# Yxxxb/LAVT-RS

Measured on NVIDIA B200. Metric: LAVT-RS fwd clips/s (8x384^2), higher is better.
Workload: dtype bf16

## Files before the change

### include/lavt_b200.h

```cpp
#ifndef LAVT_B200_H_
#define LAVT_B200_H_

#include <stdint.h>

#ifdef __cplusplus
extern "C" {
#endif

#define LAVT_ABI_VERSION 4

#define LAVT_ERR_SHAPE 1
#define LAVT_ERR_CUDA 2
#define LAVT_ERR_ARCH 3

enum { LAVT_ACT_NONE = 0, LAVT_ACT_GELU = 1, LAVT_ACT_RELU = 2, LAVT_ACT_TANH = 3, LAVT_ACT_SIGMOID = 4 };

typedef struct lavt_win_geom {
  int32_t B, D, H, W;
  int32_t wd, wh, ww;
  int32_t sd, sh, sw;
  int32_t nwd, nwh, nww;
  int32_t N;
  int32_t Wd, Wh, Ww;
} lavt_win_geom_t;

typedef struct lavt_epilogue {
  const float* cscale;
  const float* bias;
  int32_t act;
  int32_t ldm;
  const void* mul;
  const float* resid;
// ... 4 lines not shown
  const lavt_win_geom_t* win;
  const float* rscale;
  int32_t rscale_rows;
  int32_t pre_mode;
  void* out_pre;
} lavt_epilogue_t;

const char* lavt_last_error(void);
int lavt_abi_version(void);
int lavt_check_device(void);

int lavt_gemm_bf16(const void* A, int64_t lda, const void* Wt, int64_t ldw, int32_t M, int32_t N, int32_t K,
                   const lavt_epilogue_t* epi, void* stream);

int lavt_conv3x3_bf16(const void* x_nhwc, int64_t ldx, int32_t n_img, int32_t H, int32_t W, int32_t Cin,
                      const void* Wt, int32_t Cout, const lavt_epilogue_t* epi, void* stream);

int lavt_conv3d_bf16(const void* x_ndhwc, int64_t ldx, int32_t n_clip, int32_t D, int32_t H, int32_t W, int32_t Cin,
                     const void* Wt, int32_t Cout, const lavt_epilogue_t* epi, void* stream);


int lavt_layernorm_rows(const float* x, int64_t ldx, int64_t M, int32_t C, const float* gamma, const float* beta,
                        float eps, void* out_bf16, float* out_f32, void* stream);

int lavt_layernorm_window_gather(const float* x, int32_t C, const lavt_win_geom_t* geom, const float* gamma,
                                 const float* beta, float eps, void* out_bf16, void* stream);

int lavt_patch_merge_layernorm(const float* x, int32_t B, int32_t D, int32_t H, int32_t W, int32_t C,
                               const float* gamma, const float* beta, float eps, void* out_bf16, void* stream);

int lavt_patch_embed_im2col(const float* x, int64_t stride_b, int64_t stride_c, int64_t stride_t, int32_t B, int32_t T,
                            int32_t H, int32_t W, void* out_bf16, void* stream);

int lavt_window_attention(const void* qkv, const float* table_t, int32_t L, int32_t nH, const lavt_win_geom_t* geom,
                          void* out_bf16, void* stream);
int lavt_window_attention_lse(const void* qkv, const float* table_t, int32_t L, int32_t nH, const lavt_win_geom_t* geom, void* out_bf16,
                              float* lse, void* stream);
int lavt_window_attention_has_lse(const lavt_win_geom_t* geom, int32_t L, int32_t nH);
int lavt_set_attention_impl(int32_t impl);

int64_t lavt_instnorm_workspace_floats(int32_t B, int64_t n, int32_t C);
int lavt_instnorm_stats(const float* x, int32_t B, int64_t n, int32_t C, float eps, float* stats,
                        float* workspace, void* stream);
int lavt_pwam_kv(const float* l, const float* mask, const float* wk, const float* bk, const float* wv, const float* bv,
                 float* k, float* v, int32_t B, int32_t Nl, int32_t Lin, int32_t C, void* stream);
int lavt_lang_project(const float* l, const float* mask, const float* w0, const float* b0, const float* w2, const float* b2, float* stats,
// ... 157 lines not shown
```

### lavt_rs_b200/_cabi.py

```python
from __future__ import annotations

import ctypes as C
import os
from typing import Optional

import torch

_PKG = os.path.dirname(os.path.abspath(__file__))
LIB_PATH = os.environ.get("LAVT_LIB_PATH") or os.path.join(_PKG, "_lib", "liblavt_b200.so")

ACT_NONE, ACT_GELU, ACT_RELU, ACT_TANH, ACT_SIGMOID = 0, 1, 2, 3, 4


class WinGeom(C.Structure):
    _fields_ = [(n, C.c_int32) for n in
                ("B", "D", "H", "W", "wd", "wh", "ww", "sd", "sh", "sw",
                 "nwd", "nwh", "nww", "N", "Wd", "Wh", "Ww")]

    def rows(self) -> int:
        return self.B * self.nwd * self.nwh * self.nww * self.N

    def tokens(self) -> int:
        return self.B * self.D * self.H * self.W

# ... 15 lines not shown
    pass


_lib: Optional[C.CDLL] = None


def lib() -> C.CDLL:
    global _lib
    if _lib is not None:
        return _lib
    if not os.path.exists(LIB_PATH):
        raise LavtError(
            f"{LIB_PATH} not found: build it with `python -m lavt_rs_b200.build` "
            "(the B200 path has no CPU / PyTorch fallback)")
    l = C.CDLL(LIB_PATH)
    l.lavt_last_error.restype = C.c_char_p
    _declare(l)
    if l.lavt_abi_version() != ABI_VERSION:
        raise LavtError("liblavt_b200.so ABI version mismatch; rebuild")
    _lib = l
    return l


ABI_VERSION = 4

_i32, _i64, _f32, _vp = C.c_int32, C.c_int64, C.c_float, C.c_void_p
_EP = C.POINTER(Epilogue)
_WG = C.POINTER(WinGeom)

SIGNATURES = {
    "lavt_check_device": [],
    "lavt_gemm_bf16": [_vp, _i64, _vp, _i64, _i32, _i32, _i32, _EP, _vp],
    "lavt_gemm_bf16_smallm": [_vp, _i64, _vp, _i64, _i32, _i32, _i32, _EP, _vp, _i64, _vp],
    "lavt_conv3x3_bf16": [_vp, _i64, _i32, _i32, _i32, _i32, _vp, _i32, _EP, _vp],
    "lavt_conv3d_bf16": [_vp, _i64, _i32, _i32, _i32, _i32, _i32, _vp, _i32, _EP, _vp],
    "lavt_layernorm_rows": [_vp, _i64, _i64, _i32, _vp, _vp, _f32, _vp, _vp, _vp],
    "lavt_layernorm_window_gather": [_vp, _i32, _WG, _vp, _vp, _f32, _vp, _vp],
    "lavt_patch_merge_layernorm": [_vp, _i32, _i32, _i32, _i32, _i32, _vp, _vp, _f32, _vp, _vp],
    "lavt_patch_embed_im2col": [_vp, _i64, _i64, _i64, _i32, _i32, _i32, _i32, _vp, _vp],
    "lavt_window_attention": [_vp, _vp, _i32, _i32, _WG, _vp, _vp],
    "lavt_window_attention_lse": [_vp, _vp, _i32, _i32, _WG, _vp, _vp, _vp],
    "lavt_instnorm_stats": [_vp, _i32, _i64, _i32, _f32, _vp, _vp, _vp],
    "lavt_pwam_kv": [_vp, _vp, _vp, _vp, _vp, _vp, _vp, _vp, _i32, _i32, _i32, _i32, _vp],
    "lavt_lang_project": [_vp, _vp, _vp, _vp, _vp, _vp, _vp, _i32, _i32, _i32, _i32, _vp],
    "lavt_lang_project_bwd": [_vp, _vp, _vp, _vp, _vp, _vp, _vp, _vp, _vp, _vp, _vp, _vp, _i32, _i32, _i32, _i32, _vp],
    "lavt_pwam_attend": [_vp, _vp, _vp, _vp, _vp, _vp, _i32, _i64, _i32, _i32, _i32, _vp],
    "lavt_pwam_mul_norm": [_vp, _vp, _vp, _vp, _i32, _i64, _i32, _vp],
    "lavt_instnorm_sum2": [_vp, _vp, _vp, _vp, _vp, _i32, _i64, _i32, _vp],
    "lavt_bert_embed": [_vp, _vp, _vp, _vp, _vp, _i32, _i32, _i32, _i32, _vp],
    "lavt_bert_attention": [_vp, _vp, _vp, _i32, _i32, _i32, _i32, _vp],
    "lavt_rows_to_channels_first": [_vp, _vp, _i32, _i32, _i32, _vp],
    "lavt_split3_bf16": [_vp, _i64, _vp, _i64, _i32, _vp],
    "lavt_bert_attention_f32": [_vp, _vp, _vp, _i32, _i32, _i32, _i32, _vp],
    "lavt_upsample_concat": [_vp, _i32, _i32, _i32, _vp, _i32, _vp, _i32, _i32, _i32, _vp],
    "lavt_upconv_blend": [_vp, _i32, _i32, _i32, _vp, _vp, _vp, _vp, _i32, _i32, _i32, _vp],
    "lavt_conv1x1_logits": [_vp, _vp, _vp, _vp, _i64, _i32, _vp],
    "lavt_upsample_logits": [_vp, _vp, _i32, _i32, _i32, _i32, _i32, _vp],
    "lavt_nhwc_to_nchw": [_vp, _vp, _i32, _i32, _i32, _vp],
    "lavt_nchw_to_nhwc_bf16": [_vp, _vp, _i32, _i32, _i32, _vp],
# ... 254 lines not shown
    npos = n_clip * D * H * W
    TIMER.end(t0, "gemm_bf16_tc_kernel", 2.0 * npos * Cout * 27 * Cin, 2.0 * (npos * Cin + Cout * 27 * Cin + npos * Cout),
              f"conv3d {n_clip}x{D}x{H}x{W} Cin{Cin} Cout{Cout}")


def _c(t: torch.Tensor, dtype, name: str) -> torch.Tensor:
    _req(t, dtype, name)
    if not t.is_contiguous():
        raise LavtError(f"{name} must be contiguous")
    return t


def layernorm_rows(x: torch.Tensor, gamma, beta, *, out_bf16=None, out_f32=None, eps: float = 1e-5) -> None:
    _req(x, torch.float32, "x")
    M, Cn = x.shape
    for t, dt, nm in ((out_bf16, torch.bfloat16, "out_bf16"), (out_f32, torch.float32, "out_f32")):
        if t is not None:
            _c(t, dt, nm)
    check(lib().lavt_layernorm_rows(x.data_ptr(), x.stride(0), M, Cn, _c(gamma, torch.float32, "gamma").data_ptr(),
                                    _c(beta, torch.float32, "beta").data_ptr(), eps, ptr(out_bf16), ptr(out_f32),
                                    stream_ptr()), "lavt_layernorm_rows")


def layernorm_window_gather(x: torch.Tensor, geom: WinGeom, gamma, beta, out_bf16: torch.Tensor, eps: float = 1e-5) -> None:
    _c(x, torch.float32, "x")
    Cn = x.shape[-1]
    if x.numel() != geom.tokens() * Cn or out_bf16.numel() != geom.rows() * Cn:
        raise LavtError("window gather: tensor sizes do not match the geometry")
    check(lib().lavt_layernorm_window_gather(x.data_ptr(), Cn, C.byref(geom), _c(gamma, torch.float32, "gamma").data_ptr(),
                                             _c(beta, torch.float32, "beta").data_ptr(), eps,
                                             _c(out_bf16, torch.bfloat16, "out").data_ptr(), stream_ptr()),
          "lavt_layernorm_window_gather")


def patch_merge_layernorm(x: torch.Tensor, B, D, H, W, gamma, beta, out_bf16: torch.Tensor, eps: float = 1e-5) -> None:
    _c(x, torch.float32, "x")
    Cn = x.shape[-1]
    check(lib().lavt_patch_merge_layernorm(x.data_ptr(), B, D, H, W, Cn, _c(gamma, torch.float32, "gamma").data_ptr(),
                                           _c(beta, torch.float32, "beta").data_ptr(), eps,
                                           _c(out_bf16, torch.bfloat16, "out").data_ptr(), stream_ptr()),
          "lavt_patch_merge_layernorm")


def patch_embed_im2col(x: torch.Tensor, out_bf16: torch.Tensor) -> None:
    _req(x, torch.float32, "x")
    B, Cin, T, H, W = x.shape
# ... 725 lines not shown
```

### lavt_rs_b200/csrc/cabi.cu

```cuda
#include "../../include/lavt_b200.h"
#include "common.cuh"
#include "gemm_tc.cuh"
#include "kernels.cuh"

#include <cstring>

namespace lavt {
const char* last_error();
int gemm_dispatch(const void* A, long long lda, const void* Bw, long long ldb, const GemmParams& p,
                  cudaStream_t stream);

static_assert(sizeof(lavt_win_geom_t) == sizeof(WinGeom), "public/private window geometry mismatch");

static int fill_epilogue(GemmParams& p, const lavt_epilogue_t* e) {
  LAVT_REQUIRE(e != nullptr, "epilogue pointer is NULL");
  p.cscale = e->cscale;
  p.bias = e->bias;
  p.act = e->act;
  p.mul = static_cast<const __nv_bfloat16*>(e->mul);
  p.ldm = e->ldm;
  p.mul_act = e->mul_act;
  p.out_pre = static_cast<__nv_bfloat16*>(e->out_pre);
  p.pre_mode = e->pre_mode;
  LAVT_REQUIRE(e->pre_mode == 0 || (e->pre_mode == 1 && e->out_pre && e->act == LAVT_ACT_GELU),
// ... 87 lines not shown
  p.M = n_clip * D * H * W; p.N = Cout; p.K = 27 * Cin;
  int rc = fill_epilogue(p, epi);
  if (rc) return rc;
  LAVT_REQUIRE(p.rowmap == ROWMAP_IDENTITY, "conv3d: window row map not applicable");
  p.rowmap = ROWMAP_CONV;
  p.cH = H; p.cW = W; p.cCin = Cin; p.taps = 27; p.cD = D;
  conv_pick_tile(p, H, W);
  return gemm_dispatch(x_ndhwc, ldx, Wt, 27LL * Cin, p, static_cast<cudaStream_t>(stream));
}

static inline cudaStream_t S(void* s) { return static_cast<cudaStream_t>(s); }
static inline const __nv_bfloat16* CB(const void* p) { return static_cast<const __nv_bfloat16*>(p); }
static inline __nv_bfloat16* MB(void* p) { return static_cast<__nv_bfloat16*>(p); }

int lavt_layernorm_rows(const float* x, int64_t ldx, int64_t M, int32_t C, const float* gamma, const float* beta,
                        float eps, void* out_bf16, float* out_f32, void* stream) {
  LnParams p;
  std::memset(&p, 0, sizeof(p));
  p.x = x; p.ldx = ldx; p.gamma = gamma; p.beta = beta; p.out_bf16 = MB(out_bf16); p.out_f32 = out_f32;
  p.M = M; p.C = C; p.eps = eps;
  return ln_rows_dispatch(MODE_IDENTITY, p, S(stream));
}

int lavt_layernorm_window_gather(const float* x, int32_t C, const lavt_win_geom_t* geom, const float* gamma,
                                 const float* beta, float eps, void* out_bf16, void* stream) {
  LAVT_REQUIRE(geom != nullptr, "window gather: geometry is NULL");
  LnParams p;
  std::memset(&p, 0, sizeof(p));
  std::memcpy(&p.win, geom, sizeof(WinGeom));
  p.x = x; p.ldx = C; p.gamma = gamma; p.beta = beta; p.out_bf16 = MB(out_bf16);
  p.M = 1LL * geom->B * geom->nwd * geom->nwh * geom->nww * geom->N; p.C = C; p.eps = eps;
  return ln_rows_dispatch(MODE_WINDOW, p, S(stream));
}

int lavt_patch_merge_layernorm(const float* x, int32_t B, int32_t D, int32_t H, int32_t W, int32_t C,
                               const float* gamma, const float* beta, float eps, void* out_bf16, void* stream) {
  LnParams p;
  std::memset(&p, 0, sizeof(p));
  p.x = x; p.ldx = C; p.gamma = gamma; p.beta = beta; p.out_bf16 = MB(out_bf16);
  p.M = 1LL * B * D * ((H + 1) / 2) * ((W + 1) / 2); p.C = C; p.eps = eps;
  p.mB = B; p.mD = D; p.mH = H; p.mW = W;
  return ln_rows_dispatch(MODE_MERGE, p, S(stream));
}

int lavt_patch_embed_im2col(const float* x, int64_t stride_b, int64_t stride_c, int64_t stride_t, int32_t B, int32_t T,
                            int32_t H, int32_t W, void* out_bf16, void* stream) {
// ... 443 lines not shown
```

### lavt_rs_b200/csrc/common.cuh

```cuda
#pragma once

#include <cuda.h>
#include <cuda_bf16.h>
#include <cuda_runtime.h>
#include <stdint.h>
#include <string.h>

#define LAVT_OK 0
#define LAVT_ERR_SHAPE 1
#define LAVT_ERR_CUDA 2
#define LAVT_ERR_ARCH 3

namespace lavt {

void set_last_error(const char* fmt, ...);
int check_cuda(cudaError_t e, const char* what);
#define LAVT_CUDA(call)                                   \
  do {                                                    \
    int _rc = ::lavt::check_cuda((call), #call);          \
    if (_rc != LAVT_OK) return _rc;                       \
  } while (0)
#define LAVT_LAUNCH_CHECK(name)                           \
  do {                                                    \
    int _rc = ::lavt::check_cuda(cudaGetLastError(), name); \
// ... 67 lines not shown
#pragma unroll
  for (int o = 16; o > 0; o >>= 1) v += __shfl_xor_sync(0xffffffffu, v, o);
  return v;
}
__device__ __forceinline__ float warp_max(float v) {
#pragma unroll
  for (int o = 16; o > 0; o >>= 1) v = fmaxf(v, __shfl_xor_sync(0xffffffffu, v, o));
  return v;
}

__device__ __forceinline__ uint32_t pack_bf16x2(float lo, float hi) {
  __nv_bfloat162 v = __floats2bfloat162_rn(lo, hi);
  return *reinterpret_cast<uint32_t*>(&v);
}
__device__ __forceinline__ float2 unpack_bf16x2(uint32_t u) {
  __nv_bfloat162 v = *reinterpret_cast<__nv_bfloat162*>(&u);
  return __bfloat1622float2(v);
}

__device__ __forceinline__ float gelu_erf(float x) {
  return 0.5f * x * (1.0f + erff(x * 0.70710678118654752440f));
}

__device__ __forceinline__ void mbar_init(uint64_t* bar, uint32_t count) {
  asm volatile("mbarrier.init.shared::cta.b64 [%0], %1;" ::"r"(smem_u32(bar)), "r"(count));
}
__device__ __forceinline__ void fence_mbar_init() {
  asm volatile("fence.mbarrier_init.release.cluster;" ::: "memory");
}
__device__ __forceinline__ void mbar_expect_tx(uint64_t* bar, uint32_t bytes) {
  asm volatile("mbarrier.arrive.expect_tx.shared::cta.b64 _, [%0], %1;" ::"r"(smem_u32(bar)),
               "r"(bytes)
               : "memory");
}
__device__ __forceinline__ void mbar_arrive(uint64_t* bar) {
  asm volatile("mbarrier.arrive.shared::cta.b64 _, [%0];" ::"r"(smem_u32(bar)) : "memory");
}
__device__ __forceinline__ bool mbar_try_wait(uint64_t* bar, uint32_t parity) {
  uint32_t ok;
  asm volatile(
      "{\n\t"
      ".reg .pred P;\n\t"
      "mbarrier.try_wait.parity.shared::cta.b64 P, [%1], %2, %3;\n\t"
      "selp.u32 %0, 1, 0, P;\n\t"
      "}\n"
      : "=r"(ok)
// ... 242 lines not shown
```

### lavt_rs_b200/csrc/gemm_tc.cu

```cuda
#include "common.cuh"
#include "gemm_tc.cuh"

#include <cstdio>
#include <cstdlib>
#include <cstring>

namespace lavt {

constexpr int GEMM_BM = 128;
constexpr int GEMM_BK = 64;

template <int GEMM_BN, int GEMM_STAGES, int EPI_WGS, int CTA2 = 0>
struct GemmSmem {
  static constexpr int A_BYTES = GEMM_BM * GEMM_BK * 2;
  static constexpr int B_BYTES = (CTA2 ? GEMM_BN / 2 : GEMM_BN) * GEMM_BK * 2;
  static constexpr int STAGE_BYTES = A_BYTES + B_BYTES;
  static constexpr int RING_BYTES = GEMM_STAGES * STAGE_BYTES;
  static constexpr int BAR_OFF = RING_BYTES;
  static constexpr int VEC_OFF = BAR_OFF + 256;
  static constexpr int VEC_TILE_BYTES = EPI_WGS * 2 * GEMM_BN * 4;
  static constexpr int TOTAL = VEC_OFF + VEC_TILE_BYTES + 1024 ;
  static constexpr int THREADS = 128 + 128 * EPI_WGS;
  static constexpr int MIN_CTAS = (EPI_WGS == 1) ? 2 : 1;
  static constexpr int ACC = (MIN_CTAS == 2) ? 2 : 512 / GEMM_BN;
};

__device__ __forceinline__ float ex2_approx(float x) {
  float y;
  asm("ex2.approx.ftz.f32 %0, %1;" : "=f"(y) : "f"(x));
  return y;
}
__device__ __forceinline__ float rcp_approx(float x) {
  float y;
  asm("rcp.approx.ftz.f32 %0, %1;" : "=f"(y) : "f"(x));
  return y;
}
__device__ __forceinline__ uint64_t pk2(float lo, float hi) {
  uint64_t r;
  asm("mov.b64 %0, {%1, %2};" : "=l"(r) : "f"(lo), "f"(hi));
  return r;
}
__device__ __forceinline__ void upk2(uint64_t v, float& lo, float& hi) { asm("mov.b64 {%0, %1}, %2;" : "=f"(lo), "=f"(hi) : "l"(v)); }
__device__ __forceinline__ uint64_t fma2(uint64_t a, uint64_t b, uint64_t c) {
  uint64_t r;
  asm("fma.rn.f32x2 %0, %1, %2, %3;" : "=l"(r) : "l"(a), "l"(b), "l"(c));
  return r;
}
__device__ __forceinline__ uint64_t mul2(uint64_t a, uint64_t b) {
  uint64_t r;
  asm("mul.rn.f32x2 %0, %1, %2;" : "=l"(r) : "l"(a), "l"(b));
  return r;
}
__device__ __forceinline__ void gelu_erf2(float& x0, float& x1) {
  const uint64_t x = pk2(x0, x1);
  float z0, z1;
  upk2(mul2(x, pk2(0.70710678118654752f, 0.70710678118654752f)), z0, z1);
  z0 = fminf(fmaxf(z0, -3.0f), 3.0f);
  z1 = fminf(fmaxf(z1, -3.0f), 3.0f);
  const uint64_t z = pk2(z0, z1);
  const uint64_t t = mul2(z, z);
  constexpr float K = 1.0000220904f;
  uint64_t p = pk2(4.0742095563e-08f * K, 4.0742095563e-08f * K);
  p = fma2(p, t, pk2(-1.9448222676e-06f * K, -1.9448222676e-06f * K));
  p = fma2(p, t, pk2(4.1060515983e-05f * K, 4.1060515983e-05f * K));
  p = fma2(p, t, pk2(-5.1103678896e-04f * K, -5.1103678896e-04f * K));
  p = fma2(p, t, pk2(4.2354270142e-03f * K, 4.2354270142e-03f * K));
  p = fma2(p, t, pk2(-2.5102860078e-02f * K, -2.5102860078e-02f * K));
  p = fma2(p, t, pk2(1.1107933337e-01f * K, 1.1107933337e-01f * K));
  p = fma2(p, t, pk2(-3.7531487405e-01f * K, -3.7531487405e-01f * K));
  p = fma2(p, t, pk2(1.1282684285e+00f * K, 1.1282684285e+00f * K));
  const uint64_t e = mul2(z, p);
  const uint64_t hx = mul2(x, pk2(0.5f, 0.5f));
  upk2(fma2(hx, e, hx), x0, x1);
}
__device__ __forceinline__ void gelu_both2(float& x0, float& x1, float& d0, float& d1) {
  const uint64_t x = pk2(x0, x1);
  float z0, z1;
  upk2(mul2(x, pk2(0.70710678118654752f, 0.70710678118654752f)), z0, z1);
  const uint64_t zz = pk2(z0, z1);
  float q0, q1;
  upk2(mul2(zz, zz), q0, q1);
  const float e0 = ex2_approx(-1.4426950408889634f * q0), e1 = ex2_approx(-1.4426950408889634f * q1);
  z0 = fminf(fmaxf(z0, -3.0f), 3.0f);
  z1 = fminf(fmaxf(z1, -3.0f), 3.0f);
  const uint64_t z = pk2(z0, z1);
  const uint64_t t = mul2(z, z);
  constexpr float K = 1.0000220904f;
  uint64_t p = pk2(4.0742095563e-08f * K, 4.0742095563e-08f * K);
  p = fma2(p, t, pk2(-1.9448222676e-06f * K, -1.9448222676e-06f * K));
  p = fma2(p, t, pk2(4.1060515983e-05f * K, 4.1060515983e-05f * K));
  p = fma2(p, t, pk2(-5.1103678896e-04f * K, -5.1103678896e-04f * K));
  p = fma2(p, t, pk2(4.2354270142e-03f * K, 4.2354270142e-03f * K));
  p = fma2(p, t, pk2(-2.5102860078e-02f * K, -2.5102860078e-02f * K));
  p = fma2(p, t, pk2(1.1107933337e-01f * K, 1.1107933337e-01f * K));
  p = fma2(p, t, pk2(-3.7531487405e-01f * K, -3.7531487405e-01f * K));
  p = fma2(p, t, pk2(1.1282684285e+00f * K, 1.1282684285e+00f * K));
  const uint64_t Phi = fma2(mul2(z, p), pk2(0.5f, 0.5f), pk2(0.5f, 0.5f));
  const uint64_t xs = mul2(x, pk2(0.3989422804014327f, 0.3989422804014327f));
  upk2(fma2(xs, pk2(e0, e1), Phi), d0, d1);
  upk2(mul2(x, Phi), x0, x1);
}
__device__ __forceinline__ void gelu_grad2(float& x0, float& x1) {
  float d0, d1;
  gelu_both2(x0, x1, d0, d1);
  x0 = d0;
  x1 = d1;
}
__device__ __forceinline__ void ldg_v8(uint32_t* r, const void* p) {
  asm volatile("ld.global.v8.b32 {%0, %1, %2, %3, %4, %5, %6, %7}, [%8];"
               : "=r"(r[0]), "=r"(r[1]), "=r"(r[2]), "=r"(r[3]), "=r"(r[4]), "=r"(r[5]), "=r"(r[6]), "=r"(r[7])
               : "l"(p));
}
__device__ __forceinline__ void stg_v8(void* p, const uint32_t* r) {
  asm volatile("st.global.v8.b32 [%0], {%1, %2, %3, %4, %5, %6, %7, %8};" ::"l"(p), "r"(r[0]), "r"(r[1]), "r"(r[2]),
               "r"(r[3]), "r"(r[4]), "r"(r[5]), "r"(r[6]), "r"(r[7])
               : "memory");
}
__device__ __forceinline__ float tanh_fast(float x) {
  const float e = ex2_approx(x * 2.8853900817779268f);
  return fmaf(-2.0f, rcp_approx(e + 1.0f), 1.0f);
}

template <int GEMM_BN, int GEMM_STAGES, int EPI_WGS, int CTA2 = 0, int SIMPLE = 0>
__global__ void __launch_bounds__(GemmSmem<GEMM_BN, GEMM_STAGES, EPI_WGS, CTA2>::THREADS, GemmSmem<GEMM_BN, GEMM_STAGES, EPI_WGS, CTA2>::MIN_CTAS)
gemm_bf16_tc_kernel(const __grid_constant__ CUtensorMap tmA, const __grid_constant__ CUtensorMap tmB,
                    const GemmParams p, const int m_tiles, const int vec_all, long long* const trace_buf) {
  using L = GemmSmem<GEMM_BN, GEMM_STAGES, EPI_WGS, CTA2>;
  const int crank = CTA2 ? static_cast<int>(cluster_ctarank()) : 0;
  const int wid0 = CTA2 ? static_cast<int>(blockIdx.x >> 1) : static_cast<int>(blockIdx.x);
  const int wstep = CTA2 ? static_cast<int>(gridDim.x >> 1) : static_cast<int>(gridDim.x);
  extern __shared__ uint8_t smem_raw[];
  uint8_t* smem = smem_raw + ((1024u - (smem_u32(smem_raw) & 1023u)) & 1023u);
  uint64_t* full_bar = reinterpret_cast<uint64_t*>(smem + L::BAR_OFF);
  uint64_t* empty_bar = full_bar + GEMM_STAGES;
  constexpr int ACC = L::ACC;
  uint64_t* tmem_full_bar = empty_bar + GEMM_STAGES;
  uint64_t* tmem_empty_bar = tmem_full_bar + ACC;
  uint32_t* tmem_ptr_smem = reinterpret_cast<uint32_t*>(tmem_empty_bar + ACC);

  const int warp = threadIdx.x >> 5;
// ... 568 lines not shown
```

### lavt_rs_b200/csrc/kernels.cuh

```cuda
#pragma once
#include "common.cuh"
#include "geom.cuh"

namespace lavt {

enum { MODE_IDENTITY = 0, MODE_WINDOW = 1, MODE_MERGE = 2 };

struct LnParams {
  const float* x;
  long long ldx;
  const float* gamma;
  const float* beta;
  __nv_bfloat16* out_bf16;
  float* out_f32;
  long long M;
  int C;
  float eps;
  WinGeom win;
  int mB, mD, mH, mW;
};
int ln_rows_dispatch(int mode, const LnParams& p, cudaStream_t st);
int im2col_patch4_dispatch(const float* x, long long sB, long long sC, long long sT, __nv_bfloat16* out, int B, int T, int H,
                           int W, cudaStream_t st);
long long colstats_workspace_floats(int B, long long n, int C);
// ... 99 lines not shown
int pwam_kv_bwd_dispatch(const float* dkbuf, const float* dvbuf, const float* mask, const float* l, const float* wk, const float* wv,
                         float* dwk, float* dbk, float* dwv, float* dbv, float* dl, int B, int Nl, int NlPad, int Lin, int C, int heads,
                         cudaStream_t st);
int gate_elem_dispatch(int mode, const __nv_bfloat16* a, const __nv_bfloat16* b, const float* f, const float* f2, __nv_bfloat16* out_bf16,
                       float* out_f32, long long count, cudaStream_t st);

int pwam_kv_dispatch(const float* l, const float* mask, const float* wk, const float* bk, const float* wv, const float* bv,
                     float* k, float* v, int B, int Nl, int Lin, int C, cudaStream_t st);
int lang_project_dispatch(const float* l, const float* mask, const float* w0, const float* b0, const float* w2, const float* b2,
                          float* stats, int B, int Nl, int Lin, int C, cudaStream_t st);
int pwam_core_dispatch(const float* qpre, const float* stats, const float* k, const float* v, const float* mask,
                       __nv_bfloat16* o, int B, long long n, int C, int Nl, int heads, cudaStream_t st);

int bert_embed_dispatch(const long long* ids, const float* word, const float* pos, const float* type0, float* out, int B, int Nl,
                        int H, int vocab, cudaStream_t st);
int bert_attention_dispatch(const __nv_bfloat16* qkv, const float* mask, __nv_bfloat16* out, int B, int Nl, int H, int heads,
                            cudaStream_t st);
int split3_bf16_dispatch(const float* x, long long ldx, __nv_bfloat16* out, long long M, int Kd, cudaStream_t st);
int bert_attention_f32_dispatch(const float* qkv, const float* mask, float* out, int B, int Nl, int H, int heads, cudaStream_t st);
int rows_to_cf_dispatch(const float* in, float* out, int B, int Nl, int C, cudaStream_t st);

int upsample_concat_dispatch(const __nv_bfloat16* prev, int ph, int pw, int C1, const __nv_bfloat16* skip, int C2,
                             __nv_bfloat16* out, int n_img, int H, int W, cudaStream_t st);
int upconv_blend_dispatch(const __nv_bfloat16* Z, int h, int w, int hid, const float* P, const float* s, const float* b,
                          __nv_bfloat16* out, int n_img, int H, int W, cudaStream_t st);
int conv1x1_logits_dispatch(const __nv_bfloat16* y, const float* w, const float* b, float* out, long long npix, int C,
                            cudaStream_t st);
int upsample_logits_dispatch(const float* in, float* out, int n_img, int h, int w, int H, int W, cudaStream_t st);
int nhwc_to_nchw_dispatch(const float* in, float* out, int n_img, int P, int C, cudaStream_t st);
int nchw_to_nhwc_bf16_dispatch(const float* in, __nv_bfloat16* out, int n_img, int P, int C, cudaStream_t st);

}
```

### lavt_rs_b200/engine.py

```python
from __future__ import annotations

from typing import Dict, Optional, Sequence, Tuple

import torch

from . import _cabi as K
from .geometry import window_geometry

LAUNCHES = 0
PRECISION = "bf16"


def set_precision(mode: str) -> str:
    global PRECISION
    if mode not in ("bf16", "fp32"):
        raise ValueError("precision must be 'bf16' or 'fp32'")
    prev, PRECISION = PRECISION, mode
    return prev


def _count(n: int = 1) -> None:
    global LAUNCHES
    LAUNCHES += n

# ... 73 lines not shown
    if PRECISION == "fp32":
        return _swin_block_fp32(x, blk, geom, ws, xb_out)

    qkv_w = pw.get("qkv_w", [blk.attn.qkv.weight], lambda: _bf16(blk.attn.qkv.weight))
    def _qscale():
        s = torch.ones(3 * C, device=dev, dtype=torch.float32)
        s[:C] = hd ** -0.5 * 1.4426950408889634
        b = _f32(blk.attn.qkv.bias) * s if blk.attn.qkv.bias is not None else torch.zeros(3 * C, device=dev)
        return s, b
    qkv_s, qkv_b = pw.get("qkv_sb", [blk.attn.qkv.weight] + ([blk.attn.qkv.bias] if blk.attn.qkv.bias is not None else []), _qscale)
    proj_w = pw.get("proj_w", [blk.attn.proj.weight], lambda: _bf16(blk.attn.proj.weight))
    fc1_w = pw.get("fc1_w", [blk.mlp.fc1.weight], lambda: _bf16(blk.mlp.fc1.weight))
    fc2_w = pw.get("fc2_w", [blk.mlp.fc2.weight], lambda: _bf16(blk.mlp.fc2.weight))
    table_t = pw.get("table_t", [blk.attn.relative_position_bias_table],
                     lambda: _f32(blk.attn.relative_position_bias_table.t()))

    xw = ws.get("xw", (rows, C), torch.bfloat16, dev)
    K.layernorm_window_gather(x, geom, blk.norm1.weight, blk.norm1.bias, xw, eps=blk.norm1.eps)
    qkv = ws.get("qkv", (rows, 3 * C), torch.bfloat16, dev)
    K.gemm_bf16(xw, qkv_w, cscale=qkv_s, bias=qkv_b, out_bf16=qkv)
    att = ws.get("att", (rows, C), torch.bfloat16, dev)
    K.window_attention(qkv, table_t, geom, att)
    K.gemm_bf16(att, proj_w, bias=blk.attn.proj.bias.detach(), resid=x, out_f32=x, win=geom)
    h1 = ws.get("ln2", (n, C), torch.bfloat16, dev)
    K.layernorm_rows(x, blk.norm2.weight, blk.norm2.bias, out_bf16=h1, eps=blk.norm2.eps)
    hid = ws.get("hid", (n, fc1_w.shape[0]), torch.bfloat16, dev)
    K.gemm_bf16(h1, fc1_w, bias=blk.mlp.fc1.bias.detach(), act=K.ACT_GELU, out_bf16=hid)
    K.gemm_bf16(hid, fc2_w, bias=blk.mlp.fc2.bias.detach(), resid=x, out_f32=x, out_bf16=xb_out)
    _count(7)


def _swin_block_fp32(x: torch.Tensor, blk, geom, ws: Workspace, xb_out: Optional[torch.Tensor]) -> None:
    n, C = x.shape
    dev = x.device
    rows, nH = geom.rows(), blk.num_heads
    hd = C // nH
    s = torch.ones(3 * C, device=dev, dtype=torch.float32)
    s[:C] = hd ** -0.5 * 1.4426950408889634
    qb = _f32(blk.attn.qkv.bias) * s if blk.attn.qkv.bias is not None else torch.zeros(3 * C, device=dev)
    xw = ws.get("xw32", (rows, C), torch.float32, dev)
    K.layernorm_window_gather_f32(x, geom, blk.norm1.weight, blk.norm1.bias, xw, eps=blk.norm1.eps)
    qkv = ws.get("qkv32", (rows, 3 * C), torch.float32, dev)
    K.gemm_f32_ref(xw, _f32(blk.attn.qkv.weight), cscale=s, bias=qb, out_f32=qkv)
    att = ws.get("att32", (rows, C), torch.float32, dev)
    K.window_attention_f32_ref(qkv, _f32(blk.attn.relative_position_bias_table.t()), geom, att)
    K.gemm_f32_ref(att, _f32(blk.attn.proj.weight), bias=blk.attn.proj.bias.detach(), resid=x, out_f32=x, win=geom)
    h1 = ws.get("ln2_32", (n, C), torch.float32, dev)
    K.layernorm_rows(x, blk.norm2.weight, blk.norm2.bias, out_f32=h1, eps=blk.norm2.eps)
    hid = ws.get("hid32", (n, blk.mlp.fc1.weight.shape[0]), torch.float32, dev)
    K.gemm_f32_ref(h1, _f32(blk.mlp.fc1.weight), bias=blk.mlp.fc1.bias.detach(), act=K.ACT_GELU, out_f32=hid)
    K.gemm_f32_ref(hid, _f32(blk.mlp.fc2.weight), bias=blk.mlp.fc2.bias.detach(), resid=x, out_f32=x, out_bf16=xb_out)
# ... 690 lines not shown
```

Baseline: 298.1.

## Fuse Swin MLP LayerNorm, fc1+GELU, fc2 and residual into one tcgen05 kernel

Adds a persistent warp-specialized kernel for C=256 Swin blocks. It computes LayerNorm2 into shared memory, runs fc1 into TMEM, applies GELU and feeds the hidden tile back from TMEM as the A operand of fc2, then adds bias and residual in place. This removes the global round-trip of the 4C-wide hidden activation and the LN output, and drops two launches per block. The price is a complex pipeline with a 640-thread, single-CTA-per-SM configuration, and only the C=256 stage uses it.

```diff
diff --git a/include/lavt_b200.h b/include/lavt_b200.h
--- a/include/lavt_b200.h
+++ b/include/lavt_b200.h
@@ -7,7 +7,7 @@
 extern "C" {
 #endif
 
-#define LAVT_ABI_VERSION 4
+#define LAVT_ABI_VERSION 5
 
 #define LAVT_ERR_SHAPE 1
 #define LAVT_ERR_CUDA 2
@@ -58,6 +58,9 @@
 
 int lavt_layernorm_rows(const float* x, int64_t ldx, int64_t M, int32_t C, const float* gamma, const float* beta,
                         float eps, void* out_bf16, float* out_f32, void* stream);
+
+int lavt_swin_mlp(float* x, int64_t M, int32_t C, int32_t H, const float* ln_w, const float* ln_b, float eps, const void* w1_bf16,
+                  const float* b1, const void* w2_bf16, const float* b2, void* xb_out, void* stream);
 
 int lavt_layernorm_window_gather(const float* x, int32_t C, const lavt_win_geom_t* geom, const float* gamma,
                                  const float* beta, float eps, void* out_bf16, void* stream);
diff --git a/lavt_rs_b200/_cabi.py b/lavt_rs_b200/_cabi.py
--- a/lavt_rs_b200/_cabi.py
+++ b/lavt_rs_b200/_cabi.py
@@ -61,7 +61,7 @@
     return l
 
 
-ABI_VERSION = 4
+ABI_VERSION = 5
 
 _i32, _i64, _f32, _vp = C.c_int32, C.c_int64, C.c_float, C.c_void_p
 _EP = C.POINTER(Epilogue)
@@ -74,6 +74,7 @@
     "lavt_conv3x3_bf16": [_vp, _i64, _i32, _i32, _i32, _i32, _vp, _i32, _EP, _vp],
     "lavt_conv3d_bf16": [_vp, _i64, _i32, _i32, _i32, _i32, _i32, _vp, _i32, _EP, _vp],
     "lavt_layernorm_rows": [_vp, _i64, _i64, _i32, _vp, _vp, _f32, _vp, _vp, _vp],
+    "lavt_swin_mlp": [_vp, _i64, _i32, _i32, _vp, _vp, _f32, _vp, _vp, _vp, _vp, _vp, _vp],
     "lavt_layernorm_window_gather": [_vp, _i32, _WG, _vp, _vp, _f32, _vp, _vp],
     "lavt_patch_merge_layernorm": [_vp, _i32, _i32, _i32, _i32, _i32, _vp, _vp, _f32, _vp, _vp],
     "lavt_patch_embed_im2col": [_vp, _i64, _i64, _i64, _i32, _i32, _i32, _i32, _vp, _vp],
@@ -374,6 +375,24 @@
                                     stream_ptr()), "lavt_layernorm_rows")
 
 
+def swin_mlp(x: torch.Tensor, ln_w, ln_b, eps: float, w1: torch.Tensor, b1, w2: torch.Tensor, b2, *, xb_out=None) -> None:
+    _c(x, torch.float32, "x")
+    M, Cn = x.shape
+    Hn = _c(w1, torch.bfloat16, "w1").shape[0]
+    if tuple(w1.shape) != (Hn, Cn) or tuple(_c(w2, torch.bfloat16, "w2").shape) != (Cn, Hn):
+        raise LavtError(f"swin_mlp: w1 {tuple(w1.shape)} / w2 {tuple(w2.shape)} do not match C = {Cn}")
+    for t, n in ((b1, Hn), (b2, Cn)):
+        if t is not None and (_c(t, torch.float32, "bias").numel() != n):
+            raise LavtError("swin_mlp: bias size mismatch")
+    if xb_out is not None and tuple(_c(xb_out, torch.bfloat16, "xb_out").shape) != (M, Cn):
+        raise LavtError("swin_mlp: xb_out must be bf16 [M, C]")
+    t0 = TIMER.begin()
+    check(lib().lavt_swin_mlp(x.data_ptr(), M, Cn, Hn, _c(ln_w, torch.float32, "ln_w").data_ptr(), _c(ln_b, torch.float32, "ln_b").data_ptr(),
+                              eps, w1.data_ptr(), ptr(b1), w2.data_ptr(), ptr(b2), ptr(xb_out), stream_ptr()), "lavt_swin_mlp")
+    TIMER.end(t0, "swin_mlp_tc_kernel", 4.0 * M * Cn * Hn, 8.0 * M * Cn + 4.0 * Hn * Cn + (2.0 * M * Cn if xb_out is not None else 0.0),
+              f"M{M} C{Cn} H{Hn}")
+
+
 def layernorm_window_gather(x: torch.Tensor, geom: WinGeom, gamma, beta, out_bf16: torch.Tensor, eps: float = 1e-5) -> None:
     _c(x, torch.float32, "x")
     Cn = x.shape[-1]
diff --git a/lavt_rs_b200/csrc/cabi.cu b/lavt_rs_b200/csrc/cabi.cu
--- a/lavt_rs_b200/csrc/cabi.cu
+++ b/lavt_rs_b200/csrc/cabi.cu
@@ -133,6 +133,11 @@
   return ln_rows_dispatch(MODE_IDENTITY, p, S(stream));
 }
 
+int lavt_swin_mlp(float* x, int64_t M, int32_t C, int32_t H, const float* ln_w, const float* ln_b, float eps, const void* w1_bf16,
+                  const float* b1, const void* w2_bf16, const float* b2, void* xb_out, void* stream) {
+  return swin_mlp_dispatch(x, M, C, H, ln_w, ln_b, eps, CB(w1_bf16), b1, CB(w2_bf16), b2, MB(xb_out), S(stream));
+}
+
 int lavt_layernorm_window_gather(const float* x, int32_t C, const lavt_win_geom_t* geom, const float* gamma,
                                  const float* beta, float eps, void* out_bf16, void* stream) {
   LAVT_REQUIRE(geom != nullptr, "window gather: geometry is NULL");
diff --git a/lavt_rs_b200/csrc/common.cuh b/lavt_rs_b200/csrc/common.cuh
--- a/lavt_rs_b200/csrc/common.cuh
+++ b/lavt_rs_b200/csrc/common.cuh
@@ -113,6 +113,55 @@
   return 0.5f * x * (1.0f + erff(x * 0.70710678118654752440f));
 }
 
+__device__ __forceinline__ uint64_t pk2(float lo, float hi) {
+  uint64_t r;
+  asm("mov.b64 %0, {%1, %2};" : "=l"(r) : "f"(lo), "f"(hi));
+  return r;
+}
+__device__ __forceinline__ void upk2(uint64_t v, float& lo, float& hi) { asm("mov.b64 {%0, %1}, %2;" : "=f"(lo), "=f"(hi) : "l"(v)); }
+__device__ __forceinline__ uint64_t fma2(uint64_t a, uint64_t b, uint64_t c) {
+  uint64_t r;
+  asm("fma.rn.f32x2 %0, %1, %2, %3;" : "=l"(r) : "l"(a), "l"(b), "l"(c));
+  return r;
+}
+__device__ __forceinline__ uint64_t mul2(uint64_t a, uint64_t b) {
+  uint64_t r;
+  asm("mul.rn.f32x2 %0, %1, %2;" : "=l"(r) : "l"(a), "l"(b));
+  return r;
+}
+__device__ __forceinline__ void gelu_erf2(float& x0, float& x1) {
+  const uint64_t x = pk2(x0, x1);
+  float z0, z1;
+  upk2(mul2(x, pk2(0.70710678118654752f, 0.70710678118654752f)), z0, z1);
+  z0 = fminf(fmaxf(z0, -3.0f), 3.0f);
+  z1 = fminf(fmaxf(z1, -3.0f), 3.0f);
+  const uint64_t z = pk2(z0, z1);
+  const uint64_t t = mul2(z, z);
+  constexpr float K = 1.0000220904f;
+  uint64_t p = pk2(4.0742095563e-08f * K, 4.0742095563e-08f * K);
+  p = fma2(p, t, pk2(-1.9448222676e-06f * K, -1.9448222676e-06f * K));
+  p = fma2(p, t, pk2(4.1060515983e-05f * K, 4.1060515983e-05f * K));
+  p = fma2(p, t, pk2(-5.1103678896e-04f * K, -5.1103678896e-04f * K));
+  p = fma2(p, t, pk2(4.2354270142e-03f * K, 4.2354270142e-03f * K));
+  p = fma2(p, t, pk2(-2.5102860078e-02f * K, -2.5102860078e-02f * K));
+  p = fma2(p, t, pk2(1.1107933337e-01f * K, 1.1107933337e-01f * K));
+  p = fma2(p, t, pk2(-3.7531487405e-01f * K, -3.7531487405e-01f * K));
+  p = fma2(p, t, pk2(1.1282684285e+00f * K, 1.1282684285e+00f * K));
+  const uint64_t e = mul2(z, p);
+  const uint64_t hx = mul2(x, pk2(0.5f, 0.5f));
+  upk2(fma2(hx, e, hx), x0, x1);
+}
+
+__device__ __forceinline__ void ldg_v8(uint32_t* r, const void* p) {
+  asm volatile("ld.global.v8.b32 {%0, %1, %2, %3, %4, %5, %6, %7}, [%8];"
+               : "=r"(r[0]), "=r"(r[1]), "=r"(r[2]), "=r"(r[3]), "=r"(r[4]), "=r"(r[5]), "=r"(r[6]), "=r"(r[7])
+               : "l"(p));
+}
+__device__ __forceinline__ void stg_v8(void* p, const uint32_t* r) {
+  asm volatile("st.global.v8.b32 [%0], {%1, %2, %3, %4, %5, %6, %7, %8};" ::"l"(p), "r"(r[0]), "r"(r[1]), "r"(r[2]),
+               "r"(r[3]), "r"(r[4]), "r"(r[5]), "r"(r[6]), "r"(r[7])
+               : "memory");
+}
 __device__ __forceinline__ void mbar_init(uint64_t* bar, uint32_t count) {
   asm volatile("mbarrier.init.shared::cta.b64 [%0], %1;" ::"r"(smem_u32(bar)), "r"(count));
 }
diff --git a/lavt_rs_b200/csrc/gemm_tc.cu b/lavt_rs_b200/csrc/gemm_tc.cu
--- a/lavt_rs_b200/csrc/gemm_tc.cu
+++ b/lavt_rs_b200/csrc/gemm_tc.cu
@@ -34,44 +34,6 @@
   float y;
   asm("rcp.approx.ftz.f32 %0, %1;" : "=f"(y) : "f"(x));
   return y;
-}
-__device__ __forceinline__ uint64_t pk2(float lo, float hi) {
-  uint64_t r;
-  asm("mov.b64 %0, {%1, %2};" : "=l"(r) : "f"(lo), "f"(hi));
-  return r;
-}
-__device__ __forceinline__ void upk2(uint64_t v, float& lo, float& hi) { asm("mov.b64 {%0, %1}, %2;" : "=f"(lo), "=f"(hi) : "l"(v)); }
-__device__ __forceinline__ uint64_t fma2(uint64_t a, uint64_t b, uint64_t c) {
-  uint64_t r;
-  asm("fma.rn.f32x2 %0, %1, %2, %3;" : "=l"(r) : "l"(a), "l"(b), "l"(c));
-  return r;
-}
-__device__ __forceinline__ uint64_t mul2(uint64_t a, uint64_t b) {
-  uint64_t r;
-  asm("mul.rn.f32x2 %0, %1, %2;" : "=l"(r) : "l"(a), "l"(b));
-  return r;
-}
-__device__ __forceinline__ void gelu_erf2(float& x0, float& x1) {
-  const uint64_t x = pk2(x0, x1);
-  float z0, z1;
-  upk2(mul2(x, pk2(0.70710678118654752f, 0.70710678118654752f)), z0, z1);
-  z0 = fminf(fmaxf(z0, -3.0f), 3.0f);
-  z1 = fminf(fmaxf(z1, -3.0f), 3.0f);
-  const uint64_t z = pk2(z0, z1);
-  const uint64_t t = mul2(z, z);
-  constexpr float K = 1.0000220904f;
-  uint64_t p = pk2(4.0742095563e-08f * K, 4.0742095563e-08f * K);
-  p = fma2(p, t, pk2(-1.9448222676e-06f * K, -1.9448222676e-06f * K));
-  p = fma2(p, t, pk2(4.1060515983e-05f * K, 4.1060515983e-05f * K));
-  p = fma2(p, t, pk2(-5.1103678896e-04f * K, -5.1103678896e-04f * K));
-  p = fma2(p, t, pk2(4.2354270142e-03f * K, 4.2354270142e-03f * K));
-  p = fma2(p, t, pk2(-2.5102860078e-02f * K, -2.5102860078e-02f * K));
-  p = fma2(p, t, pk2(1.1107933337e-01f * K, 1.1107933337e-01f * K));
-  p = fma2(p, t, pk2(-3.7531487405e-01f * K, -3.7531487405e-01f * K));
-  p = fma2(p, t, pk2(1.1282684285e+00f * K, 1.1282684285e+00f * K));
-  const uint64_t e = mul2(z, p);
-  const uint64_t hx = mul2(x, pk2(0.5f, 0.5f));
-  upk2(fma2(hx, e, hx), x0, x1);
 }
 __device__ __forceinline__ void gelu_both2(float& x0, float& x1, float& d0, float& d1) {
   const uint64_t x = pk2(x0, x1);
@@ -106,16 +68,6 @@
   x0 = d0;
   x1 = d1;
 }
-__device__ __forceinline__ void ldg_v8(uint32_t* r, const void* p) {
-  asm volatile("ld.global.v8.b32 {%0, %1, %2, %3, %4, %5, %6, %7}, [%8];"
-               : "=r"(r[0]), "=r"(r[1]), "=r"(r[2]), "=r"(r[3]), "=r"(r[4]), "=r"(r[5]), "=r"(r[6]), "=r"(r[7])
-               : "l"(p));
-}
-__device__ __forceinline__ void stg_v8(void* p, const uint32_t* r) {
-  asm volatile("st.global.v8.b32 [%0], {%1, %2, %3, %4, %5, %6, %7, %8};" ::"l"(p), "r"(r[0]), "r"(r[1]), "r"(r[2]),
-               "r"(r[3]), "r"(r[4]), "r"(r[5]), "r"(r[6]), "r"(r[7])
-               : "memory");
-}
 __device__ __forceinline__ float tanh_fast(float x) {
   const float e = ex2_approx(x * 2.8853900817779268f);
   return fmaf(-2.0f, rcp_approx(e + 1.0f), 1.0f);
diff --git a/lavt_rs_b200/csrc/kernels.cuh b/lavt_rs_b200/csrc/kernels.cuh
--- a/lavt_rs_b200/csrc/kernels.cuh
+++ b/lavt_rs_b200/csrc/kernels.cuh
@@ -145,6 +145,8 @@
 
 int upsample_concat_dispatch(const __nv_bfloat16* prev, int ph, int pw, int C1, const __nv_bfloat16* skip, int C2,
                              __nv_bfloat16* out, int n_img, int H, int W, cudaStream_t st);
+int swin_mlp_dispatch(float* x, long long M, int C, int H, const float* ln_w, const float* ln_b, float eps, const __nv_bfloat16* w1,
+                      const float* b1, const __nv_bfloat16* w2, const float* b2, __nv_bfloat16* xb_out, cudaStream_t st);
 int upconv_blend_dispatch(const __nv_bfloat16* Z, int h, int w, int hid, const float* P, const float* s, const float* b,
                           __nv_bfloat16* out, int n_img, int H, int W, cudaStream_t st);
 int conv1x1_logits_dispatch(const __nv_bfloat16* y, const float* w, const float* b, float* out, long long npix, int C,
diff --git a/lavt_rs_b200/csrc/swin_mlp_tc.cu b/lavt_rs_b200/csrc/swin_mlp_tc.cu
--- /dev/null
+++ b/lavt_rs_b200/csrc/swin_mlp_tc.cu
@@ -0,0 +1,372 @@
+#include "attn_tc_ptx.cuh"
+#include "kernels.cuh"
+
+namespace lavt {
+
+template <int C>
+struct MlpCfg {
+  static constexpr int HID = 4 * C;
+  static constexpr int NJ = HID / 128;
+  static constexpr int KP = C / 64;
+  static constexpr int NO = 256 / C;
+  static_assert(NO >= 1 && NO <= 2, "o_empty holds two barriers");
+  static constexpr int STAGES = 5;
+  static constexpr int A_BYTES = 128 * C * 2;
+  static constexpr int PIECE = 128 * 64 * 2;
+  static constexpr int RING_OFF = 2 * A_BYTES;
+  static constexpr int BAR_OFF = RING_OFF + STAGES * PIECE;
+  static constexpr int SMEM = BAR_OFF + 256 + 1024;
+  static constexpr int THREADS = 640;
+  static constexpr int RB = 2;
+};
+
+__device__ __forceinline__ void bulk_prefetch_l2(const void* p, uint32_t bytes) {
+  asm volatile("cp.async.bulk.prefetch.L2.global [%0], %1;" ::"l"(reinterpret_cast<uint64_t>(p)), "r"(bytes) : "memory");
+}
+
+template <int C>
+__global__ void __launch_bounds__(640, 1)
+swin_mlp_tc_kernel(const __grid_constant__ CUtensorMap tmW1, const __grid_constant__ CUtensorMap tmW2, float* __restrict__ x,
+                   __nv_bfloat16* __restrict__ xb_out, const float* __restrict__ ln_w, const float* __restrict__ ln_b, const float eps,
+                   const float* __restrict__ b1, const float* __restrict__ b2, const long long M, const int m_tiles) {
+  using L = MlpCfg<C>;
+  extern __shared__ uint8_t smem_raw[];
+  uint8_t* smem = smem_raw + ((1024u - (smem_u32(smem_raw) & 1023u)) & 1023u);
+  uint64_t* full_bar = reinterpret_cast<uint64_t*>(smem + L::BAR_OFF);
+  uint64_t* empty_bar = full_bar + L::STAGES;
+  uint64_t* a_full = empty_bar + L::STAGES;
+  uint64_t* s_full = a_full + 2;
+  uint64_t* h_full = s_full + 2;
+  uint64_t* o_full = h_full + 2;
+  uint64_t* o_empty = o_full + 2;
+  uint32_t* tmem_ptr_smem = reinterpret_cast<uint32_t*>(o_empty + 2);
+
+  const int warp = threadIdx.x >> 5;
+  const int lane = threadIdx.x & 31;
+  const int n_local = (m_tiles - static_cast<int>(blockIdx.x) + static_cast<int>(gridDim.x) - 1) / static_cast<int>(gridDim.x);
+  const int G = n_local * L::NJ;
+
+  if (warp == 0 && lane == 0) {
+    tma_prefetch_desc(&tmW1);
+    tma_prefetch_desc(&tmW2);
+  }
+  if (warp == 1 && lane == 0) {
+    for (int s = 0; s < L::STAGES; ++s) {
+      mbar_init(&full_bar[s], 1);
+      mbar_init(&empty_bar[s], 1);
+    }
+    for (int i = 0; i < 2; ++i) {
+      mbar_init(&a_full[i], 4);
+      mbar_init(&s_full[i], 1);
+      mbar_init(&h_full[i], 4);
+      mbar_init(&o_full[i], 1);
+      mbar_init(&o_empty[i], 4);
+    }
+    fence_mbar_init();
+  }
+  if (warp == 2) tmem_alloc(tmem_ptr_smem, 512);
+  pdl_wait();
+  pdl_launch_dependents();
+  tc_fence_before();
+  __syncthreads();
+  tc_fence_after();
+  auto tmem_base_of = [&]() { return *reinterpret_cast<volatile uint32_t*>(tmem_ptr_smem); };
+
+  if (warp == 0) {
+    if (lane == 0) {
+      int it = 0;
+      auto load = [&](const CUtensorMap* tm, int k0, int r0) {
+        const int s = it % L::STAGES;
+        mbar_wait(&empty_bar[s], ((it / L::STAGES) & 1) ^ 1);
+        mbar_expect_tx(&full_bar[s], L::PIECE);
+        tma_load_2d(smem + L::RING_OFF + s * L::PIECE, tm, &full_bar[s], k0, r0);
+        ++it;
+      };
+      auto load_s = [&](int g) {
+        const int j = g % L::NJ;
+        for (int kp = 0; kp < L::KP; ++kp) load(&tmW1, kp * 64, j * 128);
+      };
+      auto load_f = [&](int g) {
+        const int j = g % L::NJ;
+        for (int kh = 0; kh < 2; ++kh)
+          for (int nh = 0; nh < C / 128; ++nh) load(&tmW2, j * 128 + kh * 64, nh * 128);
+      };
+      if (G > 0) load_s(0);
+      for (int g = 0; g < G; ++g) {
+        if (g + 1 < G) load_s(g + 1);
+        load_f(g);
+      }
+    }
+  } else if (warp == 1) {
+    if (lane == 0) {
+      constexpr uint32_t idesc = make_idesc_bf16_f32(128, 128);
+      const uint32_t tmem_base = tmem_base_of();
+      int it = 0;
+      auto issue_s = [&](int g) {
+        const int lt = g / L::NJ, j = g - lt * L::NJ, b = g & 1;
+        if (j == 0) {
+          mbar_wait(&a_full[lt & 1], (lt >> 1) & 1);
+          tc_fence_after();
+        }
+        const uint32_t tmem_s = tmem_base + 256 + b * 128;
+        const uint32_t a_base = smem_u32(smem + (lt & 1) * L::A_BYTES);
+        for (int kp = 0; kp < L::KP; ++kp, ++it) {
+          const int s = it % L::STAGES;
+          mbar_wait(&full_bar[s], (it / L::STAGES) & 1);
+          tc_fence_after();
+          const uint64_t da = make_kmajor_sw128_desc(a_base + kp * L::PIECE);
+          const uint64_t db = make_kmajor_sw128_desc(smem_u32(smem + L::RING_OFF + s * L::PIECE));
+#pragma unroll
+          for (int k = 0; k < 4; ++k) umma_bf16_ss(tmem_s, da + 2 * k, db + 2 * k, idesc, (kp | k) != 0);
+          umma_commit(&empty_bar[s]);
+        }
+        umma_commit(&s_full[b]);
+      };
+      auto issue_f = [&](int g) {
+        const int lt = g / L::NJ, j = g - lt * L::NJ, b = g & 1;
+        mbar_wait(&h_full[b], (g >> 1) & 1);
+        tc_fence_after();
+        const int ob = lt % L::NO;
+        if (j == 0) {
+          mbar_wait(&o_empty[ob], ((lt / L::NO) & 1) ^ 1);
+          tc_fence_after();
+        }
+        const uint32_t tmem_h = tmem_base + 256 + b * 128;
+        const uint32_t tmem_o = tmem_base + ob * C;
+        for (int kh = 0; kh < 2; ++kh) {
+          for (int nh = 0; nh < C / 128; ++nh, ++it) {
+            const int s = it % L::STAGES;
+            mbar_wait(&full_bar[s], (it / L::STAGES) & 1);
+            tc_fence_after();
+            const uint64_t db = make_kmajor_sw128_desc(smem_u32(smem + L::RING_OFF + s * L::PIECE));
+#pragma unroll
+            for (int k = 0; k < 4; ++k)
+              umma_bf16_ts(tmem_o + nh * 128, tmem_h + kh * 32 + 8 * k, db + 2 * k, idesc, (j | kh | k) != 0);
+            umma_commit(&empty_bar[s]);
+          }
+        }
+        if (j == L::NJ - 1) umma_commit(&o_full[lt & 1]);
+      };
+      if (G > 0) issue_s(0);
+      for (int g = 0; g < G; ++g) {
+        if (g + 1 < G) issue_s(g + 1);
+        issue_f(g);
+      }
+    }
+  } else if (warp >= 12) {
+    const int b = (warp - 12) >> 2;
+    const int ew = warp & 3;
+    const uint32_t tmem_base = tmem_base_of();
+    const uint32_t tb = tmem_base + 256 + b * 128 + (static_cast<uint32_t>(ew * 32) << 16);
+    for (int g = b; g < G; g += 2) {
+      const int j = g % L::NJ;
+      mbar_wait(&s_full[b], (g >> 1) & 1);
+      tc_fence_after();
+#pragma unroll 1
+      for (int c = 0; c < 4; ++c) {
+        uint32_t v[32];
+        tmem_ld_32x32b_x32(tb + c * 32, v);
+        tmem_ld_wait();
+        float f[32];
+        if (b1) {
+          const float4* bi4 = reinterpret_cast<const float4*>(b1 + j * 128 + c * 32);
+#pragma unroll
+          for (int q = 0; q < 8; ++q) {
+            const float4 bi = __ldg(bi4 + q);
+            f[4 * q] = __uint_as_float(v[4 * q]) + bi.x;
+            f[4 * q + 1] = __uint_as_float(v[4 * q + 1]) + bi.y;
+            f[4 * q + 2] = __uint_as_float(v[4 * q + 2]) + bi.z;
+            f[4 * q + 3] = __uint_as_float(v[4 * q + 3]) + bi.w;
+          }
+        } else {
+#pragma unroll
+          for (int i = 0; i < 32; ++i) f[i] = __uint_as_float(v[i]);
+        }
+        uint32_t u[16];
+#pragma unroll
+        for (int i = 0; i < 16; ++i) {
+          gelu_erf2(f[2 * i], f[2 * i + 1]);
+          u[i] = pack_bf16x2(f[2 * i], f[2 * i + 1]);
+        }
+        tmem_st_x16(tb + c * 16, u);
+      }
+      tmem_st_wait();
+      tc_fence_before();
+      __syncwarp();
+      if (lane == 0) mbar_arrive(&h_full[b]);
+    }
+  } else if (warp >= 4) {
+    const int k = (warp - 4) >> 2;
+    const int wl = warp & 3;
+    constexpr int NV = C / 128;
+    const float inv_c = 1.0f / static_cast<float>(C);
+    uint8_t* const abuf = smem + k * L::A_BYTES;
+    for (int lt = k; lt < n_local; lt += 2) {
+      const long long row0 = (static_cast<long long>(blockIdx.x) + static_cast<long long>(lt) * gridDim.x) * 128;
+      if (warp == 4 + 4 * k && lane == 0 && lt + 2 < n_local) {
+        const long long nrow0 = row0 + 2LL * gridDim.x * 128;
+        const long long nrows = (M - nrow0) < 128 ? (M - nrow0) : 128;
+        bulk_prefetch_l2(x + nrow0 * C, static_cast<uint32_t>(nrows * C * 4));
+      }
+      float4 gm[NV], bt[NV];
+#pragma unroll
+      for (int i = 0; i < NV; ++i) {
+        gm[i] = __ldg(reinterpret_cast<const float4*>(ln_w) + i * 32 + lane);
+        bt[i] = __ldg(reinterpret_cast<const float4*>(ln_b) + i * 32 + lane);
+      }
+#pragma unroll 1
+      for (int r0 = wl * 32; r0 < wl * 32 + 32; r0 += L::RB) {
+        float4 v[L::RB][NV];
+#pragma unroll
+        for (int rr = 0; rr < L::RB; ++rr) {
+          const long long m = row0 + r0 + rr;
+#pragma unroll
+          for (int i = 0; i < NV; ++i)
+            v[rr][i] = (m < M) ? __ldg(reinterpret_cast<const float4*>(x + m * C) + i * 32 + lane) : make_float4(0.f, 0.f, 0.f, 0.f);
+        }
+#pragma unroll
+        for (int rr = 0; rr < L::RB; ++rr) {
+          const int r = r0 + rr;
+          float s = 0.f;
+#pragma unroll
+          for (int i = 0; i < NV; ++i) s += (v[rr][i].x + v[rr][i].y) + (v[rr][i].z + v[rr][i].w);
+          const float mean = warp_sum(s) * inv_c;
+          float ss = 0.f;
+#pragma unroll
+          for (int i = 0; i < NV; ++i) {
+            const float a = v[rr][i].x - mean, bb = v[rr][i].y - mean, c = v[rr][i].z - mean, d = v[rr][i].w - mean;
+            ss += (a * a + bb * bb) + (c * c + d * d);
+          }
+          const float rstd = rsqrtf(warp_sum(ss) * inv_c + eps);
+          const bool live = row0 + r < M;
+#pragma unroll
+          for (int i = 0; i < NV; ++i) {
+            uint2 o = make_uint2(0u, 0u);
+            if (live) {
+              const float y0 = (v[rr][i].x - mean) * rstd * gm[i].x + bt[i].x;
+              const float y1 = (v[rr][i].y - mean) * rstd * gm[i].y + bt[i].y;
+              const float y2 = (v[rr][i].z - mean) * rstd * gm[i].z + bt[i].z;
+              const float y3 = (v[rr][i].w - mean) * rstd * gm[i].w + bt[i].w;
+              o = make_uint2(pack_bf16x2(y0, y1), pack_bf16x2(y2, y3));
+            }
+            const int col = i * 128 + lane * 4;
+            const int ch = ((col & 63) >> 3) ^ (r & 7);
+            *reinterpret_cast<uint2*>(abuf + (col >> 6) * L::PIECE + r * 128 + ch * 16 + (col & 7) * 2) = o;
+          }
+        }
+      }
+      fence_proxy_async_smem();
+      __syncwarp();
+      if (lane == 0) mbar_arrive(&a_full[k]);
+
+      const int r = wl * 32 + lane;
+      const long long m = row0 + r;
+      const bool live = m < M;
+      float* const xr = x + m * C;
+      const uint32_t tb = tmem_base_of() + (lt % L::NO) * C + (static_cast<uint32_t>(wl * 32) << 16);
+      uint32_t rr[16];
+      if (live) {
+        ldg_v8(rr, xr);
+        ldg_v8(rr + 8, xr + 8);
+      }
+      mbar_wait(&o_full[k], (lt >> 1) & 1);
+      tc_fence_after();
+#pragma unroll 1
+      for (int c = 0; c < C / 16; ++c) {
+        uint32_t v[16];
+        tmem_ld_32x32b_x16(tb + c * 16, v);
+        tmem_ld_wait();
+        if (c == C / 16 - 1) {
+          tc_fence_before();
+          __syncwarp();
+          if (lane == 0) mbar_arrive(&o_empty[lt % L::NO]);
+        }
+        uint32_t rn[16];
+        if (live && c + 1 < C / 16) {
+          ldg_v8(rn, xr + (c + 1) * 16);
+          ldg_v8(rn + 8, xr + (c + 1) * 16 + 8);
+        }
+        if (live) {
+#pragma unroll
+          for (int q = 0; q < 4; ++q) {
+            const float4 bi = b2 ? __ldg(reinterpret_cast<const float4*>(b2 + c * 16) + q) : make_float4(0.f, 0.f, 0.f, 0.f);
+            rr[4 * q] = __float_as_uint((__uint_as_float(v[4 * q]) + bi.x) + __uint_as_float(rr[4 * q]));
+            rr[4 * q + 1] = __float_as_uint((__uint_as_float(v[4 * q + 1]) + bi.y) + __uint_as_float(rr[4 * q + 1]));
+            rr[4 * q + 2] = __float_as_uint((__uint_as_float(v[4 * q + 2]) + bi.z) + __uint_as_float(rr[4 * q + 2]));
+            rr[4 * q + 3] = __float_as_uint((__uint_as_float(v[4 * q + 3]) + bi.w) + __uint_as_float(rr[4 * q + 3]));
+          }
+          stg_v8(xr + c * 16, rr);
+          stg_v8(xr + c * 16 + 8, rr + 8);
+          if (xb_out) {
+            uint32_t w[8];
+#pragma unroll
+            for (int i = 0; i < 8; ++i) w[i] = pack_bf16x2(__uint_as_float(rr[2 * i]), __uint_as_float(rr[2 * i + 1]));
+            stg_v8(xb_out + m * C + c * 16, w);
+          }
+#pragma unroll
+          for (int i = 0; i < 16; ++i) rr[i] = rn[i];
+        }
+      }
+    }
+  }
+
+  tc_fence_before();
+  __syncthreads();
+  if (warp == 2) {
+    tc_fence_after();
+    tmem_dealloc(tmem_base_of(), 512);
+  }
+}
+
+template <int C>
+static int launch_swin_mlp(const CUtensorMap& tm1, const CUtensorMap& tm2, float* x, __nv_bfloat16* xb_out, const float* ln_w,
+                           const float* ln_b, float eps, const float* b1, const float* b2, long long M, cudaStream_t st) {
+  using L = MlpCfg<C>;
+  auto kfn = swin_mlp_tc_kernel<C>;
+  static bool configured = false;
+  if (!configured) {
+    LAVT_CUDA(cudaFuncSetAttribute(kfn, cudaFuncAttributeMaxDynamicSharedMemorySize, L::SMEM));
+    configured = true;
+  }
+  static int sms = 0;
+  if (sms == 0) {
+    int dev = 0;
+    if (cudaGetDevice(&dev) != cudaSuccess || cudaDeviceGetAttribute(&sms, cudaDevAttrMultiProcessorCount, dev) != cudaSuccess || sms <= 0)
+      sms = 148;
+  }
+  const long long tiles = (M + 127) / 128;
+  LAVT_REQUIRE(tiles < (1LL << 30), "swin_mlp: too many rows (%lld)", M);
+  const int m_tiles = static_cast<int>(tiles);
+  const int grid = m_tiles < sms ? m_tiles : sms;
+  LAVT_CUDA(launch_pdl(kfn, dim3(grid), dim3(L::THREADS), L::SMEM, st, 1, tm1, tm2, x, xb_out, ln_w, ln_b, eps, b1, b2, M, m_tiles));
+  LAVT_LAUNCH_CHECK("swin_mlp_tc_kernel");
+  return LAVT_OK;
+}
+
+int swin_mlp_dispatch(float* x, long long M, int C, int H, const float* ln_w, const float* ln_b, float eps, const __nv_bfloat16* w1,
+                      const float* b1, const __nv_bfloat16* w2, const float* b2, __nv_bfloat16* xb_out, cudaStream_t st) {
+  LAVT_REQUIRE(C % 32 == 0, "swin_mlp: C=%d must be a multiple of 32", C);
+  LAVT_REQUIRE(C == 256, "swin_mlp: C=%d not supported (the fused kernel takes C = 256)", C);
+  LAVT_REQUIRE(H == 4 * C, "swin_mlp: hidden width %d must be 4 * C = %d", H, 4 * C);
+  LAVT_REQUIRE(M > 0, "swin_mlp: no rows");
+  LAVT_REQUIRE(x && ln_w && ln_b && w1 && w2, "swin_mlp: x, LayerNorm weights and fc weights are required");
+  LAVT_REQUIRE((reinterpret_cast<uintptr_t>(x) | reinterpret_cast<uintptr_t>(xb_out)) % 32 == 0 &&
+                   (reinterpret_cast<uintptr_t>(ln_w) | reinterpret_cast<uintptr_t>(ln_b) | reinterpret_cast<uintptr_t>(b1) |
+                    reinterpret_cast<uintptr_t>(b2)) % 16 == 0,
+               "swin_mlp: x / xb_out must be 32-byte and the vectors 16-byte aligned");
+  CUtensorMap tm1, tm2;
+  const uint32_t box[2] = {64, 128};
+  {
+    const uint64_t dims[2] = {(uint64_t)C, (uint64_t)H}, strides[1] = {(uint64_t)C * 2};
+    const int rc = make_tmap_bf16(&tm1, w1, 2, dims, strides, box, CU_TENSOR_MAP_SWIZZLE_128B);
+    if (rc) return rc;
+  }
+  {
+    const uint64_t dims[2] = {(uint64_t)H, (uint64_t)C}, strides[1] = {(uint64_t)H * 2};
+    const int rc = make_tmap_bf16(&tm2, w2, 2, dims, strides, box, CU_TENSOR_MAP_SWIZZLE_128B);
+    if (rc) return rc;
+  }
+  return launch_swin_mlp<256>(tm1, tm2, x, xb_out, ln_w, ln_b, eps, b1, b2, M, st);
+}
+
+}
diff --git a/lavt_rs_b200/engine.py b/lavt_rs_b200/engine.py
--- a/lavt_rs_b200/engine.py
+++ b/lavt_rs_b200/engine.py
@@ -119,11 +119,17 @@
     att = ws.get("att", (rows, C), torch.bfloat16, dev)
     K.window_attention(qkv, table_t, geom, att)
     K.gemm_bf16(att, proj_w, bias=blk.attn.proj.bias.detach(), resid=x, out_f32=x, win=geom)
+    fc1_b = blk.mlp.fc1.bias.detach() if blk.mlp.fc1.bias is not None else None
+    fc2_b = blk.mlp.fc2.bias.detach() if blk.mlp.fc2.bias is not None else None
+    if C == 256 and fc1_w.shape[0] == 4 * C:
+        K.swin_mlp(x, blk.norm2.weight, blk.norm2.bias, blk.norm2.eps, fc1_w, fc1_b, fc2_w, fc2_b, xb_out=xb_out)
+        _count(5)
+        return
     h1 = ws.get("ln2", (n, C), torch.bfloat16, dev)
     K.layernorm_rows(x, blk.norm2.weight, blk.norm2.bias, out_bf16=h1, eps=blk.norm2.eps)
     hid = ws.get("hid", (n, fc1_w.shape[0]), torch.bfloat16, dev)
-    K.gemm_bf16(h1, fc1_w, bias=blk.mlp.fc1.bias.detach(), act=K.ACT_GELU, out_bf16=hid)
-    K.gemm_bf16(hid, fc2_w, bias=blk.mlp.fc2.bias.detach(), resid=x, out_f32=x, out_bf16=xb_out)
+    K.gemm_bf16(h1, fc1_w, bias=fc1_b, act=K.ACT_GELU, out_bf16=hid)
+    K.gemm_bf16(hid, fc2_w, bias=fc2_b, resid=x, out_f32=x, out_bf16=xb_out)
     _count(7)
 
 
```

Result: no change. 299.2, median of 6 (+0.4%).
